# YonghaoHe/LFD-A-Light-and-Fast-Detector

Measured on NVIDIA H100. Metric: images/sec WIDERFACE-S inference 1280x720 batch=8 per GPU bf16, higher is better.
Workload: dtype bf16

## Files before the change

### lfd-a-light-and-fast-detector_b200/csrc/conv_umma.cu

```cuda
#include <stdlib.h>

#include <type_traits>

#include "conv_common.cuh"
#include "ptx.cuh"

namespace lfd {

static constexpr int kProdThreads = 128;
static constexpr int kConsumerThreads = 256;
static constexpr int kConvThreads = kConsumerThreads + kProdThreads;

#define LFD_LAMBDA_INLINE __attribute__((always_inline))

#ifdef LFD_B200_TRACE
#define LFD_TRACE(role, idx, slot) \
    do { if (p.trace && blockIdx.x == 0 && (idx) < 32) p.trace[((role) * 32 + (idx)) * 4 + (slot)] = clock64(); } while (0)
#define LFD_TRACE_EPI(tr, idx, slot) \
    do { if ((tr) && blockIdx.x == 0 && (idx) < 16) (tr)[(idx) * 8 + (slot)] = clock64(); } while (0)
#else
#define LFD_TRACE(role, idx, slot) ((void)0)
#define LFD_TRACE_EPI(tr, idx, slot) ((void)0)
#endif

// ... 541 lines not shown
                        const uint2 pe = *reinterpret_cast<const uint2*>(tp);
                        cp_async16_full(dst_cc + pe.y, src + pe.x);
                    }
                } else {
#pragma unroll 2
                    for (int pxi = px0; pxi < p.n_px; pxi += pstep) {
                        const PxDelta pd = delta[pxi];
                        const int y = iy0 + pd.dy, x = ix0 + pd.dx;
                        const bool ok = ((unsigned)y < (unsigned)lg.H) && ((unsigned)x < (unsigned)lg.W);
                        cp_async16(dst_cc + table[pxi].dst_off, src_cc + (ok ? (y * p.W + x) : 0) * p.Cin, ok);
                    }
                }
                cp_async_mbar_arrive(&full[s]);
                if (ptid == 0) LFD_TRACE(0, it, 2);
            }
        }
        cp_async_wait_all();
        }
    }
    LFD_TL_END(p.tl);
}

static constexpr int kS4Rows = 67, kS4Cols = 36, kS4Pix = kS4Rows * kS4Cols;
static constexpr int kS4RowBytes = kS4Cols * 8;
static constexpr int kS4PatchBytes = kS4Pix * 8;
static constexpr int kS4PerThread = (kS4Pix + kProdThreads - 1) / kProdThreads;
static constexpr int kS4Batch = 5;
static constexpr int kS4Groups = kS4Rows * 10;
static constexpr int kS4GroupsPerThread = (kS4Groups + kProdThreads - 1) / kProdThreads;
static constexpr int kS4GroupBatch = 3;
static constexpr int kS4PatchOverrun = 768;
LFD_DEVINL constexpr int s4_slot(int a, int b) {
    return ((a & 1) ? ((b & 1) ? 0 : 147) : ((b & 1) ? 291 : 446)) + (a >> 1) * 9 + (b >> 1);
}
static constexpr int kS4Lbo = 599 * 16;
static constexpr int kS4Bar = 0;
static constexpr int kS4Shift = 256;
static constexpr int kS4Staging = 2048;
static constexpr int kS4W0 = kS4Staging + 2 * 8192;
static constexpr int kS4W1 = kS4W0 + 6144;
static constexpr int kS4W2 = kS4W1 + 8192;
static constexpr int kS4W3 = kS4W2 + 73728;
static constexpr int kS4Planes = kS4W3 + 8192;
static constexpr int kS4Ring = kS4Planes + 8 * kS4Lbo;
static constexpr int kS4Smem = kS4Ring + 2 * kS4PatchBytes + kS4PatchOverrun;
static constexpr int kS4WBytes = kS4Planes - kS4W0;
static_assert(kS4Smem <= 227 * 1024, "stem4 shared memory");

LFD_DEVINL void s4_block(int i, int& a0, int& b0, bool& packed) {
    packed = i == 8 || i == 13;
    a0 = packed ? 32 : 8 * (i < 8 ? i >> 1 : i - 9);
    b0 = i < 8 ? 1 + 8 * (i & 1) : (i == 8 ? 1 : 0);
}
LFD_DEVINL void s4_run(int num_tiles, int& t0, int& t1) {
    t0 = (int)((uint64_t)blockIdx.x * (uint32_t)num_tiles / gridDim.x);
    t1 = (int)((uint64_t)(blockIdx.x + 1) * (uint32_t)num_tiles / gridDim.x);
}

LFD_DEVINL void consumers_bar_sync() { asm volatile("bar.sync 3, 256;" ::: "memory"); }

template <bool F16, bool EXT>
__global__ void __launch_bounds__(kConvThreads, 1) stem4_kernel(const __grid_constant__ UmmaConvParams p) {
    extern __shared__ __align__(1024) uint8_t smem[];
    uint64_t* full = reinterpret_cast<uint64_t*>(smem + kS4Bar);
    uint64_t* empty = full + 2;
    uint64_t* wbar = empty + 2;
    uint64_t* res_bar = wbar + 1;
    float* shifts = reinterpret_cast<float*>(smem + kS4Shift);
    pdl_launch_dependents();
    LFD_TL_BEGIN(p.tl);
    const int tid = threadIdx.x;
    const int warp = tid >> 5;
    const int lane = tid & 31;
    if (tid == 0) {
        for (int i = 0; i < 2; ++i) {
            mbar_init(&full[i], kProdThreads);
            mbar_init(&empty[i], kConsumerThreads / 32);
        }
        mbar_init(wbar, 1);
        mbar_init(&res_bar[0], 1);
        mbar_init(&res_bar[1], 1);
        fence_mbar_init();
    }
    if (tid < 256) {
        const int k = tid >> 6;
        const float* s = k == 0 ? p.shift : (k == 1 ? p.shift2 : (k == 2 ? p.shift_s2 : p.shift_s3));
        shifts[tid] = s ? round16<F16>(s[tid & 63]) : 0.f;
    }
    __syncthreads();
    const LaunchGrid lg = launch_grid<MODE_STEM4, EXT>(p);

    if (warp < kConsumerThreads / 32) {
        asm volatile("setmaxnreg.inc.sync.aligned.u32 224;");
        const int wg = warp >> 2;
        if (tid == 0) {
            mbar_arrive_expect_tx(wbar, kS4WBytes);
            auto load_w = [&](uint32_t dst, const __nv_bfloat16* src, uint32_t bytes) LFD_LAMBDA_INLINE {
                for (uint32_t off = 0; off < bytes; off += 32768)
                    bulk_g2s(smem_u32(smem) + dst + off, reinterpret_cast<const uint8_t*>(src) + off, bytes - off < 32768 ? bytes - off : 32768, wbar);
            };
            load_w(kS4W0, p.w, kS4W1 - kS4W0);
            load_w(kS4W1, p.w2, kS4W2 - kS4W1);
            load_w(kS4W2, p.w_s2, kS4W3 - kS4W2);
            load_w(kS4W3, p.w_s3, kS4Planes - kS4W3);
        }
        pdl_wait();
        mbar_wait(wbar, 0);

        EpiCtx e;
        e.stg_bytes = 8192u;
        e.nbuf = 1;
        e.stg = smem_u32(smem + kS4Staging) + (uint32_t)wg * 8192u;
        e.r0 = (warp & 3) * 16 + (lane >> 2);
        e.tq = lane & 3;
        e.wtid = tid & 127;
        e.wg = wg;
        e.lane = lane;
#ifdef LFD_B200_TRACE
        e.tr = p.trace && e.wtid == 0 ? p.trace + (3 * 32 + wg) * 4 : nullptr;
#endif
        const float* sh0 = shifts;
        const float* sh1 = shifts + 64;
        const float* sh2 = shifts + 128;
        const float* sh3 = shifts + 192;
        const uint32_t planes = smem_u32(smem + kS4Planes);
        const uint64_t adesc_stem = wgmma_desc(0, 16, 2 * kS4RowBytes);
        const uint64_t adesc_row = wgmma_desc(0, 16, 8 * 16);
        const uint64_t b0desc = wgmma_desc(smem_u32(smem + kS4W0), 64 * 16, 128);
        const uint64_t b1desc = wgmma_desc(smem_u32(smem + kS4W1), 64 * 16, 128);
        const uint64_t b2desc = wgmma_desc(smem_u32(smem + kS4W2), 64 * 16, 128);
        const uint64_t b3desc = wgmma_desc(smem_u32(smem + kS4W3), 64 * 16, 128);
        const uint64_t adesc_pl = wgmma_desc(planes + (uint32_t)wg * 8u * 144u, kS4Lbo, 144);
        const int brow = 2 * (warp & 3), bcol = lane >> 2;
        const int sh = (lane >> 3) & 1, sc = lane & 7;

        const int H1 = EXT ? (lg.H - 1) / 2 + 1 : p.H1, W1 = EXT ? (lg.W - 1) / 2 + 1 : p.W1;
        int tile0, tile1;
        s4_run(lg.num_tiles, tile0, tile1);
        uint32_t store_count = 0, res_count = 0;
        for (int tile = tile0, lt = 0; tile < tile1; ++tile, ++lt) {
            const uint32_t s = lt & 1, ph = (lt >> 1) & 1;
            const int n = fast_div(tile, lg.magic_tpi);
            const int t = tile - n * lg.tiles_per_img;
            const int ty = fast_div(t, lg.magic_tx);
            const int tx = t - ty * lg.tiles_x;
            const int oy0 = ty * 16, ox0 = tx * 8;
            const bool inherit = tile > tile0 && tx > 0, pass_on = tile + 1 < tile1 && tx + 1 < lg.tiles_x;
            if (e.wtid == 0) LFD_TRACE(1 + wg, lt, 0);
            mbar_wait(&full[s], ph);
            if (e.wtid == 0) LFD_TRACE(1 + wg, lt, 1);
            fence_proxy_async_smem();
            const uint32_t patch = smem_u32(smem + kS4Ring) + s * kS4PatchBytes;

            const int nblk = inherit ? 9 : 14, half = (nblk + 1) >> 1;
            const int first = wg ? half : 0, cnt = wg ? nblk - half : half;
#pragma unroll 1
            for (int kp = 0; kp < (cnt + 1) >> 1; ++kp) {
                int blk[2] = {first + 2 * kp, first + min(2 * kp + 1, cnt - 1)};
                float c0[2][32];
                wgmma_fence_regs<32>(c0[0]);
                wgmma_fence_regs<32>(c0[1]);
                wgmma_fence();
#pragma unroll
                for (int q = 0; q < 2; ++q) {
                    int a0, b0;
                    bool packed;
                    s4_block(blk[q], a0, b0, packed);
                    const uint32_t boff = (uint32_t)(a0 * 2 * kS4RowBytes + b0 * 16);
                    const uint64_t ad = (packed ? adesc_row : adesc_stem) + ((patch + boff) >> 4);
#pragma unroll
                    for (int kh = 0; kh < 3; ++kh)
                        wgmma_ss<64, F16>(c0[q], ad + (uint32_t)(kh * kS4RowBytes / 16), b0desc + (uint32_t)(kh * 2 * 64 * 16 / 16), kh != 0);
                }
                wgmma_commit();
                wgmma_wait<0>();
                wgmma_fence_regs<32>(c0[0]);
                wgmma_fence_regs<32>(c0[1]);
                uint32_t a1[2][16];
#pragma unroll
                for (int q = 0; q < 2; ++q)
#pragma unroll
                    for (int kk = 0; kk < 4; ++kk) {
                        const int c = 16 * kk + 2 * e.tq;
#pragma unroll
                        for (int r = 0; r < 4; ++r) {
                            const float x0 = c0[q][8 * kk + 2 * r] + sh0[c + 8 * (r >> 1)], x1 = c0[q][8 * kk + 2 * r + 1] + sh0[c + 8 * (r >> 1) + 1];
                            a1[q][4 * kk + r] = p.relu ? pack2_relu<F16>(x0, x1) : pack2<F16>(x0, x1);
                        }
                    }
                float c1[2][32];
                wgmma_fence_regs<32>(c1[0]);
                wgmma_fence_regs<32>(c1[1]);
                wgmma_fence();
                tail_mma<64, 64, F16>(c1[0], a1[0], b1desc);
                tail_mma<64, 64, F16>(c1[1], a1[1], b1desc);
                wgmma_commit();
                wgmma_wait<0>();
                wgmma_fence_regs<32>(c1[0]);
                wgmma_fence_regs<32>(c1[1]);
                float2 bv[8];
#pragma unroll
                for (int j = 0; j < 8; ++j) bv[j] = *reinterpret_cast<const float2*>(sh1 + 8 * j + 2 * e.tq);
#pragma unroll
                for (int q = 0; q < 2; ++q) {
                    int a0, b0;
                    bool packed;
                    s4_block(blk[q], a0, b0, packed);
                    if (packed && (warp & 3)) continue;
                    uint32_t v[8][2];
#pragma unroll
                    for (int h = 0; h < 2; ++h) {
                        const int a = packed ? a0 : a0 + brow + h, b = b0 + bcol + (packed ? 8 * h : 0);
                        const int y1 = 2 * oy0 - 1 + a, x1 = 2 * ox0 - 1 + b;
                        const bool in = (unsigned)y1 < (unsigned)H1 && (unsigned)x1 < (unsigned)W1;
#pragma unroll
                        for (int j = 0; j < 8; ++j) {
                            const float x0 = c1[q][4 * j + 2 * h] + bv[j].x, x1v = c1[q][4 * j + 2 * h + 1] + bv[j].y;
                            const uint32_t w = p.relu2 ? pack2_relu<F16>(x0, x1v) : pack2<F16>(x0, x1v);
                            v[j][h] = in ? w : 0u;
                        }
                    }
                    const int a = packed ? a0 : a0 + brow + sh, b = b0 + sc + (packed ? 8 * sh : 0);
                    const uint32_t addr = planes + (uint32_t)s4_slot(a, b) * 16u + (uint32_t)(lane >> 4) * kS4Lbo;
#pragma unroll
                    for (int k = 0; k < 4; ++k)
                        stmatrix_x4(addr + (uint32_t)(2 * k * kS4Lbo), v[2 * k][0], v[2 * k][1], v[2 * k + 1][0], v[2 * k + 1][1]);
                }
            }
            __syncwarp();
            if (lane == 0) mbar_arrive(&empty[s]);
            if (e.wtid == 0) LFD_TRACE(1 + wg, lt, 2);
            fence_proxy_async_smem();
            consumers_bar_sync();
            if (e.wtid == 0) LFD_TRACE(1 + wg, lt, 3);

            float acc[32];
            wgmma_fence_regs<32>(acc);
            wgmma_fence();
#pragma unroll
            for (int k16 = 0; k16 < 4; ++k16)
#pragma unroll
                for (int tap = 0; tap < 9; ++tap)
                    wgmma_ss<64, F16>(acc, adesc_pl + (uint32_t)(k16 * 2 * kS4Lbo / 16 + s4_slot(tap / 3, tap % 3)),
                                      b2desc + (uint32_t)((tap * 8 + 2 * k16) * 64 * 16 / 16), (k16 | tap) != 0);
            wgmma_commit();
            wgmma_wait<0>();
            wgmma_fence_regs<32>(acc);
            consumers_bar_sync();
            if (pass_on) {
                const int rs = lane >> 3, a = 16 * wg + brow + (rs & 1) + 8 * (rs >> 1);
                const uint32_t src = planes + (uint32_t)(lane & 7) * kS4Lbo + (uint32_t)s4_slot(a, 16) * 16u;
                sts128(src - 8u * 16u, lds128(src));
                if (wg == 1 && brow == 0 && lane < 8) {
                    const uint32_t src32 = planes + (uint32_t)lane * kS4Lbo + (uint32_t)s4_slot(32, 16) * 16u;
                    sts128(src32 - 8u * 16u, lds128(src32));
                }
                __syncwarp();
            }
#ifdef LFD_B200_TRACE
            if (e.wtid == 0 && p.trace && blockIdx.x == 0 && lt < 16) p.trace[(3 * 32 + wg + 2 * lt) * 4 + 3] = clock64();
#endif

            uint32_t a2[16];
#pragma unroll
            for (int kk = 0; kk < 4; ++kk) {
                const int c = 16 * kk + 2 * e.tq;
#pragma unroll
                for (int r = 0; r < 4; ++r) {
                    const float x0 = acc[8 * kk + 2 * r] + sh2[c + 8 * (r >> 1)], x1 = acc[8 * kk + 2 * r + 1] + sh2[c + 8 * (r >> 1) + 1];
                    a2[4 * kk + r] = p.relu_s2 ? pack2_relu<F16>(x0, x1) : pack2<F16>(x0, x1);
                }
            }
            float acc2[32];
            wgmma_fence_regs<32>(acc2);
            wgmma_fence();
            tail_mma<64, 64, F16>(acc2, a2, b3desc);
            wgmma_commit();
            wgmma_wait<0>();
            wgmma_fence_regs<32>(acc2);
            store_tile<MODE_3X3S2, 64, F16>(e, acc2, 64, sh3, (bool)p.relu_s3, false, nullptr, &p.tm_out, &p.tm_res, ox0, oy0 + wg * 8, n,
                                            true, true, &res_bar[wg], store_count, res_count);
        }
        if (e.wtid == 0) bulk_wait_all();
    } else {
        asm volatile("setmaxnreg.dec.sync.aligned.u32 56;");
        const int ptid = tid - kConsumerThreads;
        const bool u8 = p.input_format == 1;
        const int plane = p.H * p.W;
        pdl_wait();
        int tile0, tile1;
        s4_run(lg.num_tiles, tile0, tile1);
        for (int tile = tile0, lt = 0; tile < tile1; ++tile, ++lt) {
            const uint32_t s = lt & 1, ph = (lt >> 1) & 1;
            const int n = fast_div(tile, lg.magic_tpi), t = tile - n * lg.tiles_per_img;
            const int ty = fast_div(t, lg.magic_tx);
            const int iy0 = 4 * 16 * ty - 3, ix0 = 4 * 8 * (t - ty * lg.tiles_x) - 3;
            const bool interior = iy0 >= 0 && ix0 >= 0 && iy0 + kS4Rows <= lg.H && ix0 + kS4Cols <= lg.W;
            if (ptid == 0) LFD_TRACE(0, lt, 0);
            mbar_wait(&empty[s], ph ^ 1);
            if (ptid == 0) LFD_TRACE(0, lt, 1);
            const uint32_t dst0 = smem_u32(smem + kS4Ring) + s * kS4PatchBytes;
            if (p.in_words) {
#pragma unroll 1
                for (int j0 = 0; j0 < kS4GroupsPerThread; j0 += kS4GroupBatch) {
                    uint32_t wd[kS4GroupBatch][3];
                    bool ok[kS4GroupBatch];
#pragma unroll
                    for (int j = 0; j < kS4GroupBatch; ++j) {
                        const int q = ptid + (j0 + j) * kProdThreads;
                        const int r = q / 10, g = q - r * 10;
                        const int y = iy0 + r, x = ix0 - 1 + 4 * g;
                        ok[j] = q < kS4Groups && (unsigned)y < (unsigned)lg.H && (unsigned)x < (unsigned)lg.W;
                        const uint32_t* src = reinterpret_cast<const uint32_t*>(reinterpret_cast<const uint8_t*>(p.in_raw) +
                                                                                ((ptrdiff_t)n * plane + (ptrdiff_t)y * p.W + x) * 3);
#pragma unroll
                        for (int k = 0; k < 3; ++k) wd[j][k] = ok[j] ? __ldg(src + k) : 0u;
                    }
#pragma unroll
                    for (int j = 0; j < kS4GroupBatch; ++j) {
                        const int q = ptid + (j0 + j) * kProdThreads;
                        if (q >= kS4Groups) break;
                        const int r = q / 10, g = q - r * 10;
                        const int in_cols = lg.W - (ix0 - 1 + 4 * g);
                        uint32_t px[4][2];
#pragma unroll
                        for (int k = 0; k < 4; ++k) {
                            float f[3];
                            const bool okk = ok[j] && (!EXT || k < in_cols);
#pragma unroll
                            for (int c = 0; c < 3; ++c) {
                                const uint32_t byte = (wd[j][(3 * k + c) >> 2] >> (8 * ((3 * k + c) & 3))) & 0xffu;
                                f[c] = okk ? ((float)byte - 127.5f) * (1.0f / 127.5f) : 0.f;
                            }
                            px[k][0] = pack2<F16>(f[0], f[1]);
                            px[k][1] = pack2<F16>(f[2], 0.f);
                        }
                        const uint32_t d = dst0 + (uint32_t)(r * kS4RowBytes + 32 * g);
                        if (g > 0) asm volatile("st.shared.v2.b32 [%0], {%1, %2};" ::"r"(d - 8u), "r"(px[0][0]), "r"(px[0][1]) : "memory");
                        if (g < 9) {
                            asm volatile("st.shared.v4.b32 [%0], {%1, %2, %3, %4};" ::"r"(d), "r"(px[1][0]), "r"(px[1][1]), "r"(px[2][0]),
                                         "r"(px[2][1]) : "memory");
                            asm volatile("st.shared.v2.b32 [%0], {%1, %2};" ::"r"(d + 16u), "r"(px[3][0]), "r"(px[3][1]) : "memory");
                        }
                    }
                }
            } else {
#pragma unroll 1
                for (int j0 = 0; j0 < kS4PerThread; j0 += kS4Batch) {
                    uint32_t raw[kS4Batch][3];
                    bool ok[kS4Batch];
#pragma unroll
                    for (int j = 0; j < kS4Batch; ++j) {
                        const int q = ptid + (j0 + j) * kProdThreads;
                        const int r = q / kS4Cols, c = q - r * kS4Cols;
                        const int y = iy0 + r, x = ix0 + c;
                        ok[j] = q < kS4Pix && (interior || ((unsigned)y < (unsigned)lg.H && (unsigned)x < (unsigned)lg.W));
                        const ptrdiff_t pix = ok[j] ? (ptrdiff_t)n * plane + (ptrdiff_t)y * p.W + x : 0;
                        if (u8) {
                            const uint8_t* src = reinterpret_cast<const uint8_t*>(p.in_raw) + pix * 3;
                            raw[j][0] = __ldg(src); raw[j][1] = __ldg(src + 1); raw[j][2] = __ldg(src + 2);
                        } else {
                            const float* src = reinterpret_cast<const float*>(p.in_raw) + (ok[j] ? (ptrdiff_t)n * 2 * plane + pix : 0);
                            raw[j][0] = __float_as_uint(__ldg(src)); raw[j][1] = __float_as_uint(__ldg(src + plane));
                            raw[j][2] = __float_as_uint(__ldg(src + 2 * plane));
                        }
                    }
#pragma unroll
                    for (int j = 0; j < kS4Batch; ++j) {
                        const int q = ptid + (j0 + j) * kProdThreads;
                        if (q >= kS4Pix) break;
                        float f[3];
#pragma unroll
                        for (int k = 0; k < 3; ++k) {
                            f[k] = u8 ? ((float)raw[j][k] - 127.5f) * (1.0f / 127.5f) : __uint_as_float(raw[j][k]);
                            if (!ok[j]) f[k] = 0.f;
                        }
                        const uint32_t lo = pack2<F16>(f[0], f[1]), hi = pack2<F16>(f[2], 0.f);
                        asm volatile("st.shared.v2.b32 [%0], {%1, %2};" ::"r"(dst0 + q * 8), "r"(lo), "r"(hi) : "memory");
                    }
                }
            }
// ... 283 lines not shown
```

### lfd-a-light-and-fast-detector_b200/csrc/ptx.cuh

```cuda
#pragma once
#include <cuda_runtime.h>
#include <cuda_bf16.h>
#include <cuda_fp16.h>
#include <stdint.h>

namespace lfd {

#define LFD_DEVINL __device__ __forceinline__

#ifndef LFD_SPIN_LIMIT
#define LFD_SPIN_LIMIT (1u << 27)
#endif

LFD_DEVINL uint32_t smem_u32(const void* p) { return (uint32_t)__cvta_generic_to_shared(p); }

LFD_DEVINL void mbar_init(uint64_t* bar, uint32_t count) {
    asm volatile("mbarrier.init.shared::cta.b64 [%0], %1;" ::"r"(smem_u32(bar)), "r"(count));
}
LFD_DEVINL void fence_mbar_init() { asm volatile("fence.mbarrier_init.release.cluster;" ::: "memory"); }
LFD_DEVINL void mbar_arrive(uint64_t* bar) {
    asm volatile("mbarrier.arrive.shared::cta.b64 _, [%0];" ::"r"(smem_u32(bar)) : "memory");
}
LFD_DEVINL void mbar_arrive_expect_tx(uint64_t* bar, uint32_t bytes) {
    asm volatile("mbarrier.arrive.expect_tx.shared::cta.b64 _, [%0], %1;" ::"r"(smem_u32(bar)), "r"(bytes) : "memory");
// ... 81 lines not shown
LFD_DEVINL void bulk_wait_all() { asm volatile("cp.async.bulk.wait_group 0;" ::: "memory"); }
template <int N>
LFD_DEVINL void bulk_wait_read() { asm volatile("cp.async.bulk.wait_group.read %0;" ::"n"(N) : "memory"); }

LFD_DEVINL uint64_t wgmma_desc(uint32_t smem_addr, uint32_t lbo_bytes, uint32_t sbo_bytes) {
    uint64_t d = 0;
    d |= (uint64_t)((smem_addr >> 4) & 0x3FFF);
    d |= (uint64_t)((lbo_bytes >> 4) & 0x3FFF) << 16;
    d |= (uint64_t)((sbo_bytes >> 4) & 0x3FFF) << 32;
    return d;
}
LFD_DEVINL void wgmma_fence() { asm volatile("wgmma.fence.sync.aligned;" ::: "memory"); }
LFD_DEVINL void wgmma_commit() { asm volatile("wgmma.commit_group.sync.aligned;" ::: "memory"); }
template <int N>
LFD_DEVINL void wgmma_wait() { asm volatile("wgmma.wait_group.sync.aligned %0;" ::"n"(N) : "memory"); }
template <int N>
LFD_DEVINL void wgmma_fence_regs(float* d) {
#pragma unroll
    for (int i = 0; i < N; ++i) asm volatile("" : "+f"(d[i])::"memory");
}

template <int N> struct Wgmma;
template <> struct Wgmma<16> {
    template <int TA, int TB>
    static LFD_DEVINL void ss_bf16(float* d, uint64_t a, uint64_t b, uint32_t acc) {
        asm volatile("{\n\t.reg .pred p;\n\tsetp.ne.b32 p, %10, 0;\n\t"
                     "wgmma.mma_async.sync.aligned.m64n16k16.f32.bf16.bf16 {%0, %1, %2, %3, %4, %5, %6, %7}, %8, %9, p, 1, 1, %11, %12;\n\t}"
                     : "+f"(d[0]), "+f"(d[1]), "+f"(d[2]), "+f"(d[3]), "+f"(d[4]), "+f"(d[5]), "+f"(d[6]), "+f"(d[7])
                     : "l"(a), "l"(b), "r"(acc), "n"(TA), "n"(TB));
    }
    template <int TA, int TB>
    static LFD_DEVINL void ss_f16(float* d, uint64_t a, uint64_t b, uint32_t acc) {
        asm volatile("{\n\t.reg .pred p;\n\tsetp.ne.b32 p, %10, 0;\n\t"
                     "wgmma.mma_async.sync.aligned.m64n16k16.f32.f16.f16 {%0, %1, %2, %3, %4, %5, %6, %7}, %8, %9, p, 1, 1, %11, %12;\n\t}"
                     : "+f"(d[0]), "+f"(d[1]), "+f"(d[2]), "+f"(d[3]), "+f"(d[4]), "+f"(d[5]), "+f"(d[6]), "+f"(d[7])
                     : "l"(a), "l"(b), "r"(acc), "n"(TA), "n"(TB));
    }
};
template <> struct Wgmma<32> {
    template <int TA, int TB>
    static LFD_DEVINL void ss_bf16(float* d, uint64_t a, uint64_t b, uint32_t acc) {
        asm volatile("{\n\t.reg .pred p;\n\tsetp.ne.b32 p, %18, 0;\n\t"
                     "wgmma.mma_async.sync.aligned.m64n32k16.f32.bf16.bf16 {%0, %1, %2, %3, %4, %5, %6, %7, %8, %9, %10, %11, %12, %13, %14, %15}, %16, %17, p, 1, 1, %19, %20;\n\t}"
                     : "+f"(d[0]), "+f"(d[1]), "+f"(d[2]), "+f"(d[3]), "+f"(d[4]), "+f"(d[5]), "+f"(d[6]), "+f"(d[7]), "+f"(d[8]), "+f"(d[9]), "+f"(d[10]), "+f"(d[11]), "+f"(d[12]), "+f"(d[13]), "+f"(d[14]), "+f"(d[15])
                     : "l"(a), "l"(b), "r"(acc), "n"(TA), "n"(TB));
    }
    template <int TA, int TB>
    static LFD_DEVINL void ss_f16(float* d, uint64_t a, uint64_t b, uint32_t acc) {
        asm volatile("{\n\t.reg .pred p;\n\tsetp.ne.b32 p, %18, 0;\n\t"
                     "wgmma.mma_async.sync.aligned.m64n32k16.f32.f16.f16 {%0, %1, %2, %3, %4, %5, %6, %7, %8, %9, %10, %11, %12, %13, %14, %15}, %16, %17, p, 1, 1, %19, %20;\n\t}"
                     : "+f"(d[0]), "+f"(d[1]), "+f"(d[2]), "+f"(d[3]), "+f"(d[4]), "+f"(d[5]), "+f"(d[6]), "+f"(d[7]), "+f"(d[8]), "+f"(d[9]), "+f"(d[10]), "+f"(d[11]), "+f"(d[12]), "+f"(d[13]), "+f"(d[14]), "+f"(d[15])
                     : "l"(a), "l"(b), "r"(acc), "n"(TA), "n"(TB));
    }
};
template <> struct Wgmma<64> {
    template <int TA, int TB>
    static LFD_DEVINL void ss_bf16(float* d, uint64_t a, uint64_t b, uint32_t acc) {
        asm volatile("{\n\t.reg .pred p;\n\tsetp.ne.b32 p, %34, 0;\n\t"
                     "wgmma.mma_async.sync.aligned.m64n64k16.f32.bf16.bf16 {%0, %1, %2, %3, %4, %5, %6, %7, %8, %9, %10, %11, %12, %13, %14, %15, %16, %17, %18, %19, %20, %21, %22, %23, %24, %25, %26, %27, %28, %29, %30, %31}, %32, %33, p, 1, 1, %35, %36;\n\t}"
                     : "+f"(d[0]), "+f"(d[1]), "+f"(d[2]), "+f"(d[3]), "+f"(d[4]), "+f"(d[5]), "+f"(d[6]), "+f"(d[7]), "+f"(d[8]), "+f"(d[9]), "+f"(d[10]), "+f"(d[11]), "+f"(d[12]), "+f"(d[13]), "+f"(d[14]), "+f"(d[15]), "+f"(d[16]), "+f"(d[17]), "+f"(d[18]), "+f"(d[19]), "+f"(d[20]), "+f"(d[21]), "+f"(d[22]), "+f"(d[23]), "+f"(d[24]), "+f"(d[25]), "+f"(d[26]), "+f"(d[27]), "+f"(d[28]), "+f"(d[29]), "+f"(d[30]), "+f"(d[31])
                     : "l"(a), "l"(b), "r"(acc), "n"(TA), "n"(TB));
    }
    template <int TA, int TB>
    static LFD_DEVINL void ss_f16(float* d, uint64_t a, uint64_t b, uint32_t acc) {
        asm volatile("{\n\t.reg .pred p;\n\tsetp.ne.b32 p, %34, 0;\n\t"
                     "wgmma.mma_async.sync.aligned.m64n64k16.f32.f16.f16 {%0, %1, %2, %3, %4, %5, %6, %7, %8, %9, %10, %11, %12, %13, %14, %15, %16, %17, %18, %19, %20, %21, %22, %23, %24, %25, %26, %27, %28, %29, %30, %31}, %32, %33, p, 1, 1, %35, %36;\n\t}"
                     : "+f"(d[0]), "+f"(d[1]), "+f"(d[2]), "+f"(d[3]), "+f"(d[4]), "+f"(d[5]), "+f"(d[6]), "+f"(d[7]), "+f"(d[8]), "+f"(d[9]), "+f"(d[10]), "+f"(d[11]), "+f"(d[12]), "+f"(d[13]), "+f"(d[14]), "+f"(d[15]), "+f"(d[16]), "+f"(d[17]), "+f"(d[18]), "+f"(d[19]), "+f"(d[20]), "+f"(d[21]), "+f"(d[22]), "+f"(d[23]), "+f"(d[24]), "+f"(d[25]), "+f"(d[26]), "+f"(d[27]), "+f"(d[28]), "+f"(d[29]), "+f"(d[30]), "+f"(d[31])
                     : "l"(a), "l"(b), "r"(acc), "n"(TA), "n"(TB));
    }
};
template <> struct Wgmma<128> {
    template <int TA, int TB>
    static LFD_DEVINL void ss_bf16(float* d, uint64_t a, uint64_t b, uint32_t acc) {
        asm volatile("{\n\t.reg .pred p;\n\tsetp.ne.b32 p, %66, 0;\n\t"
                     "wgmma.mma_async.sync.aligned.m64n128k16.f32.bf16.bf16 {%0, %1, %2, %3, %4, %5, %6, %7, %8, %9, %10, %11, %12, %13, %14, %15, %16, %17, %18, %19, %20, %21, %22, %23, %24, %25, %26, %27, %28, %29, %30, %31, %32, %33, %34, %35, %36, %37, %38, %39, %40, %41, %42, %43, %44, %45, %46, %47, %48, %49, %50, %51, %52, %53, %54, %55, %56, %57, %58, %59, %60, %61, %62, %63}, %64, %65, p, 1, 1, %67, %68;\n\t}"
                     : "+f"(d[0]), "+f"(d[1]), "+f"(d[2]), "+f"(d[3]), "+f"(d[4]), "+f"(d[5]), "+f"(d[6]), "+f"(d[7]), "+f"(d[8]), "+f"(d[9]), "+f"(d[10]), "+f"(d[11]), "+f"(d[12]), "+f"(d[13]), "+f"(d[14]), "+f"(d[15]), "+f"(d[16]), "+f"(d[17]), "+f"(d[18]), "+f"(d[19]), "+f"(d[20]), "+f"(d[21]), "+f"(d[22]), "+f"(d[23]), "+f"(d[24]), "+f"(d[25]), "+f"(d[26]), "+f"(d[27]), "+f"(d[28]), "+f"(d[29]), "+f"(d[30]), "+f"(d[31]), "+f"(d[32]), "+f"(d[33]), "+f"(d[34]), "+f"(d[35]), "+f"(d[36]), "+f"(d[37]), "+f"(d[38]), "+f"(d[39]), "+f"(d[40]), "+f"(d[41]), "+f"(d[42]), "+f"(d[43]), "+f"(d[44]), "+f"(d[45]), "+f"(d[46]), "+f"(d[47]), "+f"(d[48]), "+f"(d[49]), "+f"(d[50]), "+f"(d[51]), "+f"(d[52]), "+f"(d[53]), "+f"(d[54]), "+f"(d[55]), "+f"(d[56]), "+f"(d[57]), "+f"(d[58]), "+f"(d[59]), "+f"(d[60]), "+f"(d[61]), "+f"(d[62]), "+f"(d[63])
                     : "l"(a), "l"(b), "r"(acc), "n"(TA), "n"(TB));
    }
    template <int TA, int TB>
    static LFD_DEVINL void ss_f16(float* d, uint64_t a, uint64_t b, uint32_t acc) {
        asm volatile("{\n\t.reg .pred p;\n\tsetp.ne.b32 p, %66, 0;\n\t"
                     "wgmma.mma_async.sync.aligned.m64n128k16.f32.f16.f16 {%0, %1, %2, %3, %4, %5, %6, %7, %8, %9, %10, %11, %12, %13, %14, %15, %16, %17, %18, %19, %20, %21, %22, %23, %24, %25, %26, %27, %28, %29, %30, %31, %32, %33, %34, %35, %36, %37, %38, %39, %40, %41, %42, %43, %44, %45, %46, %47, %48, %49, %50, %51, %52, %53, %54, %55, %56, %57, %58, %59, %60, %61, %62, %63}, %64, %65, p, 1, 1, %67, %68;\n\t}"
                     : "+f"(d[0]), "+f"(d[1]), "+f"(d[2]), "+f"(d[3]), "+f"(d[4]), "+f"(d[5]), "+f"(d[6]), "+f"(d[7]), "+f"(d[8]), "+f"(d[9]), "+f"(d[10]), "+f"(d[11]), "+f"(d[12]), "+f"(d[13]), "+f"(d[14]), "+f"(d[15]), "+f"(d[16]), "+f"(d[17]), "+f"(d[18]), "+f"(d[19]), "+f"(d[20]), "+f"(d[21]), "+f"(d[22]), "+f"(d[23]), "+f"(d[24]), "+f"(d[25]), "+f"(d[26]), "+f"(d[27]), "+f"(d[28]), "+f"(d[29]), "+f"(d[30]), "+f"(d[31]), "+f"(d[32]), "+f"(d[33]), "+f"(d[34]), "+f"(d[35]), "+f"(d[36]), "+f"(d[37]), "+f"(d[38]), "+f"(d[39]), "+f"(d[40]), "+f"(d[41]), "+f"(d[42]), "+f"(d[43]), "+f"(d[44]), "+f"(d[45]), "+f"(d[46]), "+f"(d[47]), "+f"(d[48]), "+f"(d[49]), "+f"(d[50]), "+f"(d[51]), "+f"(d[52]), "+f"(d[53]), "+f"(d[54]), "+f"(d[55]), "+f"(d[56]), "+f"(d[57]), "+f"(d[58]), "+f"(d[59]), "+f"(d[60]), "+f"(d[61]), "+f"(d[62]), "+f"(d[63])
                     : "l"(a), "l"(b), "r"(acc), "n"(TA), "n"(TB));
    }
};
template <int N> struct WgmmaRs;
template <> struct WgmmaRs<16> {
    static LFD_DEVINL void rs_bf16(float* d, const uint32_t* a, uint64_t b, uint32_t acc) {
        asm volatile("{\n\t.reg .pred p;\n\tsetp.ne.b32 p, %13, 0;\n\t"
                     "wgmma.mma_async.sync.aligned.m64n16k16.f32.bf16.bf16 {%0, %1, %2, %3, %4, %5, %6, %7}, {%8, %9, %10, %11}, %12, p, 1, 1, 0;\n\t}"
                     : "+f"(d[0]), "+f"(d[1]), "+f"(d[2]), "+f"(d[3]), "+f"(d[4]), "+f"(d[5]), "+f"(d[6]), "+f"(d[7])
                     : "r"(a[0]), "r"(a[1]), "r"(a[2]), "r"(a[3]), "l"(b), "r"(acc));
    }
    static LFD_DEVINL void rs_f16(float* d, const uint32_t* a, uint64_t b, uint32_t acc) {
        asm volatile("{\n\t.reg .pred p;\n\tsetp.ne.b32 p, %13, 0;\n\t"
                     "wgmma.mma_async.sync.aligned.m64n16k16.f32.f16.f16 {%0, %1, %2, %3, %4, %5, %6, %7}, {%8, %9, %10, %11}, %12, p, 1, 1, 0;\n\t}"
                     : "+f"(d[0]), "+f"(d[1]), "+f"(d[2]), "+f"(d[3]), "+f"(d[4]), "+f"(d[5]), "+f"(d[6]), "+f"(d[7])
                     : "r"(a[0]), "r"(a[1]), "r"(a[2]), "r"(a[3]), "l"(b), "r"(acc));
    }
};
template <> struct WgmmaRs<32> {
    static LFD_DEVINL void rs_bf16(float* d, const uint32_t* a, uint64_t b, uint32_t acc) {
        asm volatile("{\n\t.reg .pred p;\n\tsetp.ne.b32 p, %21, 0;\n\t"
                     "wgmma.mma_async.sync.aligned.m64n32k16.f32.bf16.bf16 {%0, %1, %2, %3, %4, %5, %6, %7, %8, %9, %10, %11, %12, %13, %14, %15}, {%16, %17, %18, %19}, %20, p, 1, 1, 0;\n\t}"
                     : "+f"(d[0]), "+f"(d[1]), "+f"(d[2]), "+f"(d[3]), "+f"(d[4]), "+f"(d[5]), "+f"(d[6]), "+f"(d[7]), "+f"(d[8]), "+f"(d[9]), "+f"(d[10]), "+f"(d[11]), "+f"(d[12]), "+f"(d[13]), "+f"(d[14]), "+f"(d[15])
                     : "r"(a[0]), "r"(a[1]), "r"(a[2]), "r"(a[3]), "l"(b), "r"(acc));
    }
    static LFD_DEVINL void rs_f16(float* d, const uint32_t* a, uint64_t b, uint32_t acc) {
        asm volatile("{\n\t.reg .pred p;\n\tsetp.ne.b32 p, %21, 0;\n\t"
                     "wgmma.mma_async.sync.aligned.m64n32k16.f32.f16.f16 {%0, %1, %2, %3, %4, %5, %6, %7, %8, %9, %10, %11, %12, %13, %14, %15}, {%16, %17, %18, %19}, %20, p, 1, 1, 0;\n\t}"
                     : "+f"(d[0]), "+f"(d[1]), "+f"(d[2]), "+f"(d[3]), "+f"(d[4]), "+f"(d[5]), "+f"(d[6]), "+f"(d[7]), "+f"(d[8]), "+f"(d[9]), "+f"(d[10]), "+f"(d[11]), "+f"(d[12]), "+f"(d[13]), "+f"(d[14]), "+f"(d[15])
                     : "r"(a[0]), "r"(a[1]), "r"(a[2]), "r"(a[3]), "l"(b), "r"(acc));
    }
};
template <> struct WgmmaRs<64> {
    static LFD_DEVINL void rs_bf16(float* d, const uint32_t* a, uint64_t b, uint32_t acc) {
        asm volatile("{\n\t.reg .pred p;\n\tsetp.ne.b32 p, %37, 0;\n\t"
                     "wgmma.mma_async.sync.aligned.m64n64k16.f32.bf16.bf16 {%0, %1, %2, %3, %4, %5, %6, %7, %8, %9, %10, %11, %12, %13, %14, %15, %16, %17, %18, %19, %20, %21, %22, %23, %24, %25, %26, %27, %28, %29, %30, %31}, {%32, %33, %34, %35}, %36, p, 1, 1, 0;\n\t}"
                     : "+f"(d[0]), "+f"(d[1]), "+f"(d[2]), "+f"(d[3]), "+f"(d[4]), "+f"(d[5]), "+f"(d[6]), "+f"(d[7]), "+f"(d[8]), "+f"(d[9]), "+f"(d[10]), "+f"(d[11]), "+f"(d[12]), "+f"(d[13]), "+f"(d[14]), "+f"(d[15]), "+f"(d[16]), "+f"(d[17]), "+f"(d[18]), "+f"(d[19]), "+f"(d[20]), "+f"(d[21]), "+f"(d[22]), "+f"(d[23]), "+f"(d[24]), "+f"(d[25]), "+f"(d[26]), "+f"(d[27]), "+f"(d[28]), "+f"(d[29]), "+f"(d[30]), "+f"(d[31])
                     : "r"(a[0]), "r"(a[1]), "r"(a[2]), "r"(a[3]), "l"(b), "r"(acc));
    }
    static LFD_DEVINL void rs_f16(float* d, const uint32_t* a, uint64_t b, uint32_t acc) {
        asm volatile("{\n\t.reg .pred p;\n\tsetp.ne.b32 p, %37, 0;\n\t"
                     "wgmma.mma_async.sync.aligned.m64n64k16.f32.f16.f16 {%0, %1, %2, %3, %4, %5, %6, %7, %8, %9, %10, %11, %12, %13, %14, %15, %16, %17, %18, %19, %20, %21, %22, %23, %24, %25, %26, %27, %28, %29, %30, %31}, {%32, %33, %34, %35}, %36, p, 1, 1, 0;\n\t}"
                     : "+f"(d[0]), "+f"(d[1]), "+f"(d[2]), "+f"(d[3]), "+f"(d[4]), "+f"(d[5]), "+f"(d[6]), "+f"(d[7]), "+f"(d[8]), "+f"(d[9]), "+f"(d[10]), "+f"(d[11]), "+f"(d[12]), "+f"(d[13]), "+f"(d[14]), "+f"(d[15]), "+f"(d[16]), "+f"(d[17]), "+f"(d[18]), "+f"(d[19]), "+f"(d[20]), "+f"(d[21]), "+f"(d[22]), "+f"(d[23]), "+f"(d[24]), "+f"(d[25]), "+f"(d[26]), "+f"(d[27]), "+f"(d[28]), "+f"(d[29]), "+f"(d[30]), "+f"(d[31])
                     : "r"(a[0]), "r"(a[1]), "r"(a[2]), "r"(a[3]), "l"(b), "r"(acc));
    }
};
template <> struct WgmmaRs<128> {
    static LFD_DEVINL void rs_bf16(float* d, const uint32_t* a, uint64_t b, uint32_t acc) {
        asm volatile("{\n\t.reg .pred p;\n\tsetp.ne.b32 p, %69, 0;\n\t"
                     "wgmma.mma_async.sync.aligned.m64n128k16.f32.bf16.bf16 {%0, %1, %2, %3, %4, %5, %6, %7, %8, %9, %10, %11, %12, %13, %14, %15, %16, %17, %18, %19, %20, %21, %22, %23, %24, %25, %26, %27, %28, %29, %30, %31, %32, %33, %34, %35, %36, %37, %38, %39, %40, %41, %42, %43, %44, %45, %46, %47, %48, %49, %50, %51, %52, %53, %54, %55, %56, %57, %58, %59, %60, %61, %62, %63}, {%64, %65, %66, %67}, %68, p, 1, 1, 0;\n\t}"
                     : "+f"(d[0]), "+f"(d[1]), "+f"(d[2]), "+f"(d[3]), "+f"(d[4]), "+f"(d[5]), "+f"(d[6]), "+f"(d[7]), "+f"(d[8]), "+f"(d[9]), "+f"(d[10]), "+f"(d[11]), "+f"(d[12]), "+f"(d[13]), "+f"(d[14]), "+f"(d[15]), "+f"(d[16]), "+f"(d[17]), "+f"(d[18]), "+f"(d[19]), "+f"(d[20]), "+f"(d[21]), "+f"(d[22]), "+f"(d[23]), "+f"(d[24]), "+f"(d[25]), "+f"(d[26]), "+f"(d[27]), "+f"(d[28]), "+f"(d[29]), "+f"(d[30]), "+f"(d[31]), "+f"(d[32]), "+f"(d[33]), "+f"(d[34]), "+f"(d[35]), "+f"(d[36]), "+f"(d[37]), "+f"(d[38]), "+f"(d[39]), "+f"(d[40]), "+f"(d[41]), "+f"(d[42]), "+f"(d[43]), "+f"(d[44]), "+f"(d[45]), "+f"(d[46]), "+f"(d[47]), "+f"(d[48]), "+f"(d[49]), "+f"(d[50]), "+f"(d[51]), "+f"(d[52]), "+f"(d[53]), "+f"(d[54]), "+f"(d[55]), "+f"(d[56]), "+f"(d[57]), "+f"(d[58]), "+f"(d[59]), "+f"(d[60]), "+f"(d[61]), "+f"(d[62]), "+f"(d[63])
                     : "r"(a[0]), "r"(a[1]), "r"(a[2]), "r"(a[3]), "l"(b), "r"(acc));
    }
    static LFD_DEVINL void rs_f16(float* d, const uint32_t* a, uint64_t b, uint32_t acc) {
        asm volatile("{\n\t.reg .pred p;\n\tsetp.ne.b32 p, %69, 0;\n\t"
                     "wgmma.mma_async.sync.aligned.m64n128k16.f32.f16.f16 {%0, %1, %2, %3, %4, %5, %6, %7, %8, %9, %10, %11, %12, %13, %14, %15, %16, %17, %18, %19, %20, %21, %22, %23, %24, %25, %26, %27, %28, %29, %30, %31, %32, %33, %34, %35, %36, %37, %38, %39, %40, %41, %42, %43, %44, %45, %46, %47, %48, %49, %50, %51, %52, %53, %54, %55, %56, %57, %58, %59, %60, %61, %62, %63}, {%64, %65, %66, %67}, %68, p, 1, 1, 0;\n\t}"
                     : "+f"(d[0]), "+f"(d[1]), "+f"(d[2]), "+f"(d[3]), "+f"(d[4]), "+f"(d[5]), "+f"(d[6]), "+f"(d[7]), "+f"(d[8]), "+f"(d[9]), "+f"(d[10]), "+f"(d[11]), "+f"(d[12]), "+f"(d[13]), "+f"(d[14]), "+f"(d[15]), "+f"(d[16]), "+f"(d[17]), "+f"(d[18]), "+f"(d[19]), "+f"(d[20]), "+f"(d[21]), "+f"(d[22]), "+f"(d[23]), "+f"(d[24]), "+f"(d[25]), "+f"(d[26]), "+f"(d[27]), "+f"(d[28]), "+f"(d[29]), "+f"(d[30]), "+f"(d[31]), "+f"(d[32]), "+f"(d[33]), "+f"(d[34]), "+f"(d[35]), "+f"(d[36]), "+f"(d[37]), "+f"(d[38]), "+f"(d[39]), "+f"(d[40]), "+f"(d[41]), "+f"(d[42]), "+f"(d[43]), "+f"(d[44]), "+f"(d[45]), "+f"(d[46]), "+f"(d[47]), "+f"(d[48]), "+f"(d[49]), "+f"(d[50]), "+f"(d[51]), "+f"(d[52]), "+f"(d[53]), "+f"(d[54]), "+f"(d[55]), "+f"(d[56]), "+f"(d[57]), "+f"(d[58]), "+f"(d[59]), "+f"(d[60]), "+f"(d[61]), "+f"(d[62]), "+f"(d[63])
                     : "r"(a[0]), "r"(a[1]), "r"(a[2]), "r"(a[3]), "l"(b), "r"(acc));
    }
};
template <int N, bool F16, int TA = 0, int TB = 0>
LFD_DEVINL void wgmma_ss(float* d, uint64_t a, uint64_t b, uint32_t acc) {
    if (F16) Wgmma<N>::template ss_f16<TA, TB>(d, a, b, acc);
    else Wgmma<N>::template ss_bf16<TA, TB>(d, a, b, acc);
}
template <int N, bool F16>
LFD_DEVINL void wgmma_rs(float* d, const uint32_t* a, uint64_t b, uint32_t acc) {
    if (F16) WgmmaRs<N>::rs_f16(d, a, b, acc);
    else WgmmaRs<N>::rs_bf16(d, a, b, acc);
}
LFD_DEVINL void stmatrix_x4(uint32_t addr, uint32_t r0, uint32_t r1, uint32_t r2, uint32_t r3) {
    asm volatile("stmatrix.sync.aligned.m8n8.x4.shared.b16 [%0], {%1, %2, %3, %4};" ::"r"(addr), "r"(r0), "r"(r1), "r"(r2), "r"(r3) : "memory");
}

#ifdef LFD_B200_TIMELINE
LFD_DEVINL unsigned long long globaltimer_ns() {
    unsigned long long t;
    asm volatile("mov.u64 %0, %%globaltimer;" : "=l"(t));
    return t;
}
#define LFD_TL_BEGIN(tl) do { if ((tl) && threadIdx.x == 0) atomicMin((tl), globaltimer_ns()); } while (0)
#define LFD_TL_END(tl) do { if ((tl) && threadIdx.x == 0) atomicMax((tl) + 1, globaltimer_ns()); } while (0)
#else
#define LFD_TL_BEGIN(tl) ((void)0)
#define LFD_TL_END(tl) ((void)0)
#endif
LFD_DEVINL uint32_t pack_bf16x2(float lo, float hi) {
    __nv_bfloat162 v = __floats2bfloat162_rn(lo, hi);
    return *reinterpret_cast<uint32_t*>(&v);
}
LFD_DEVINL uint32_t pack_bf16x2_relu(float lo, float hi) {
    uint32_t d;
    asm("cvt.rn.relu.bf16x2.f32 %0, %1, %2;" : "=r"(d) : "f"(hi), "f"(lo));
    return d;
}
LFD_DEVINL void sts128(uint32_t addr, uint4 v) {
    asm volatile("st.shared.v4.b32 [%0], {%1, %2, %3, %4};" ::"r"(addr), "r"(v.x), "r"(v.y), "r"(v.z), "r"(v.w) : "memory");
}
LFD_DEVINL float lds32f(uint32_t addr) {
    float v;
    asm volatile("ld.shared.f32 %0, [%1];" : "=f"(v) : "r"(addr) : "memory");
    return v;
}
LFD_DEVINL uint4 lds128(uint32_t addr) {
    uint4 v;
    asm volatile("ld.shared.v4.b32 {%0, %1, %2, %3}, [%4];" : "=r"(v.x), "=r"(v.y), "=r"(v.z), "=r"(v.w) : "r"(addr) : "memory");
    return v;
}
LFD_DEVINL float bf16_lo(uint32_t v) { return __uint_as_float(v << 16); }
LFD_DEVINL float bf16_hi(uint32_t v) { return __uint_as_float(v & 0xFFFF0000u); }
LFD_DEVINL float bf16_round(float x) { return __bfloat162float(__float2bfloat16_rn(x)); }

LFD_DEVINL uint32_t pack_f16x2(float lo, float hi) {
    uint32_t d;
    asm("cvt.rn.satfinite.f16x2.f32 %0, %1, %2;" : "=r"(d) : "f"(hi), "f"(lo));
    return d;
}
LFD_DEVINL uint32_t pack_f16x2_relu(float lo, float hi) {
    uint32_t d;
    asm("cvt.rn.relu.satfinite.f16x2.f32 %0, %1, %2;" : "=r"(d) : "f"(hi), "f"(lo));
    return d;
}
LFD_DEVINL float f16_lo(uint32_t v) { return __half2float(__ushort_as_half((unsigned short)(v & 0xFFFFu))); }
LFD_DEVINL float f16_hi(uint32_t v) { return __half2float(__ushort_as_half((unsigned short)(v >> 16))); }
template <bool F16> LFD_DEVINL uint32_t pack2(float lo, float hi) { return F16 ? pack_f16x2(lo, hi) : pack_bf16x2(lo, hi); }
template <bool F16> LFD_DEVINL uint32_t pack2_relu(float lo, float hi) { return F16 ? pack_f16x2_relu(lo, hi) : pack_bf16x2_relu(lo, hi); }
template <bool F16> LFD_DEVINL float up_lo(uint32_t v) { return F16 ? f16_lo(v) : bf16_lo(v); }
template <bool F16> LFD_DEVINL float up_hi(uint32_t v) { return F16 ? f16_hi(v) : bf16_hi(v); }
template <bool F16> LFD_DEVINL float round16(float x) { return F16 ? __half2float(__float2half_rn(x)) : bf16_round(x); }
template <bool F16> LFD_DEVINL uint32_t bits16(float x) {
    return F16 ? (uint32_t)__half_as_ushort(__float2half_rn(x)) : (uint32_t)__bfloat16_as_ushort(__float2bfloat16_rn(x));
}
LFD_DEVINL float up_lo_rt(uint32_t v, bool f16) { return f16 ? f16_lo(v) : bf16_lo(v); }
LFD_DEVINL float up_hi_rt(uint32_t v, bool f16) { return f16 ? f16_hi(v) : bf16_hi(v); }
LFD_DEVINL uint32_t pack2_rt(float lo, float hi, bool f16) { return f16 ? pack_f16x2(lo, hi) : pack_bf16x2(lo, hi); }
LFD_DEVINL float round16_rt(float x, bool f16) { return f16 ? __half2float(__float2half_rn(x)) : bf16_round(x); }

}
```

Measured before the change: 10450.

## Software-pipeline stem conv0/conv1 wgmma chain across blocks with async waits

After: 10720, median of 6. +2.6%, better.

```diff
diff --git a/lfd-a-light-and-fast-detector_b200/csrc/conv_umma.cu b/lfd-a-light-and-fast-detector_b200/csrc/conv_umma.cu
--- a/lfd-a-light-and-fast-detector_b200/csrc/conv_umma.cu
+++ b/lfd-a-light-and-fast-detector_b200/csrc/conv_umma.cu
@@ -717,61 +717,52 @@
             fence_proxy_async_smem();
             const uint32_t patch = smem_u32(smem + kS4Ring) + s * kS4PatchBytes;
 
-            const int nblk = inherit ? 9 : 14, half = (nblk + 1) >> 1;
-            const int first = wg ? half : 0, cnt = wg ? nblk - half : half;
-#pragma unroll 1
-            for (int kp = 0; kp < (cnt + 1) >> 1; ++kp) {
-                int blk[2] = {first + 2 * kp, first + min(2 * kp + 1, cnt - 1)};
-                float c0[2][32];
-                wgmma_fence_regs<32>(c0[0]);
-                wgmma_fence_regs<32>(c0[1]);
-                wgmma_fence();
-#pragma unroll
-                for (int q = 0; q < 2; ++q) {
+            const uint32_t blocks = inherit ? (wg ? 0x87654u : 0x3210u) : (wg ? 0xCB87654u : 0xDA93210u);
+            auto stem01 = [&](auto nb) LFD_LAMBDA_INLINE {
+                constexpr int NB = decltype(nb)::value;
+                static_assert(NB >= 2, "stem0/1 pipeline depth");
+                float c0[2][32], c1[2][32];
+                uint32_t a1[2][16];
+                auto issue_s0 = [&](int k) LFD_LAMBDA_INLINE {
                     int a0, b0;
                     bool packed;
-                    s4_block(blk[q], a0, b0, packed);
-                    const uint32_t boff = (uint32_t)(a0 * 2 * kS4RowBytes + b0 * 16);
-                    const uint64_t ad = (packed ? adesc_row : adesc_stem) + ((patch + boff) >> 4);
-#pragma unroll
-                    for (int kh = 0; kh < 3; ++kh)
-                        wgmma_ss<64, F16>(c0[q], ad + (uint32_t)(kh * kS4RowBytes / 16), b0desc + (uint32_t)(kh * 2 * 64 * 16 / 16), kh != 0);
-                }
-                wgmma_commit();
-                wgmma_wait<0>();
-                wgmma_fence_regs<32>(c0[0]);
-                wgmma_fence_regs<32>(c0[1]);
-                uint32_t a1[2][16];
-#pragma unroll
-                for (int q = 0; q < 2; ++q)
+                    s4_block((blocks >> 4 * k) & 15, a0, b0, packed);
+                    const uint64_t ad = (packed ? adesc_row : adesc_stem) + ((patch + (uint32_t)(a0 * 2 * kS4RowBytes + b0 * 16)) >> 4);
+                    wgmma_fence();
+                    wgmma_ss64_first<F16>(c0[k & 1], ad, b0desc);
+#pragma unroll
+                    for (int kh = 1; kh < 3; ++kh)
+                        wgmma_ss<64, F16>(c0[k & 1], ad + (uint32_t)(kh * kS4RowBytes / 16), b0desc + (uint32_t)(kh * 2 * 64 * 16 / 16), 1);
+                    wgmma_commit();
+                };
+                auto issue_s1 = [&](int k) LFD_LAMBDA_INLINE {
+                    float* c = c0[k & 1];
+                    uint32_t* a = a1[k & 1];
+                    wgmma_fence_regs<32>(c);
 #pragma unroll
                     for (int kk = 0; kk < 4; ++kk) {
-                        const int c = 16 * kk + 2 * e.tq;
+                        const int ch = 16 * kk + 2 * e.tq;
 #pragma unroll
                         for (int r = 0; r < 4; ++r) {
-                            const float x0 = c0[q][8 * kk + 2 * r] + sh0[c + 8 * (r >> 1)], x1 = c0[q][8 * kk + 2 * r + 1] + sh0[c + 8 * (r >> 1) + 1];
-                            a1[q][4 * kk + r] = p.relu ? pack2_relu<F16>(x0, x1) : pack2<F16>(x0, x1);
+                            const float x0 = c[8 * kk + 2 * r] + sh0[ch + 8 * (r >> 1)], x1 = c[8 * kk + 2 * r + 1] + sh0[ch + 8 * (r >> 1) + 1];
+                            a[4 * kk + r] = p.relu ? pack2_relu<F16>(x0, x1) : pack2<F16>(x0, x1);
                         }
                     }
-                float c1[2][32];
-                wgmma_fence_regs<32>(c1[0]);
-                wgmma_fence_regs<32>(c1[1]);
-                wgmma_fence();
-                tail_mma<64, 64, F16>(c1[0], a1[0], b1desc);
-                tail_mma<64, 64, F16>(c1[1], a1[1], b1desc);
-                wgmma_commit();
-                wgmma_wait<0>();
-                wgmma_fence_regs<32>(c1[0]);
-                wgmma_fence_regs<32>(c1[1]);
-                float2 bv[8];
-#pragma unroll
-                for (int j = 0; j < 8; ++j) bv[j] = *reinterpret_cast<const float2*>(sh1 + 8 * j + 2 * e.tq);
-#pragma unroll
-                for (int q = 0; q < 2; ++q) {
+                    wgmma_fence();
+                    wgmma_rs64_first<F16>(c1[k & 1], a, b1desc);
+#pragma unroll
+                    for (int kk = 1; kk < 4; ++kk) wgmma_rs<64, F16>(c1[k & 1], a + 4 * kk, b1desc + (uint32_t)(kk * 2 * 64 * 16 / 16), 1);
+                    wgmma_commit();
+                };
+                auto store = [&](int k) LFD_LAMBDA_INLINE {
+                    float* c = c1[k & 1];
+                    wgmma_fence_regs<32>(c);
                     int a0, b0;
                     bool packed;
-                    s4_block(blk[q], a0, b0, packed);
-                    if (packed && (warp & 3)) continue;
+                    s4_block((blocks >> 4 * k) & 15, a0, b0, packed);
+                    float2 bv[8];
+#pragma unroll
+                    for (int j = 0; j < 8; ++j) bv[j] = *reinterpret_cast<const float2*>(sh1 + 8 * j + 2 * e.tq);
                     uint32_t v[8][2];
 #pragma unroll
                     for (int h = 0; h < 2; ++h) {
@@ -780,18 +771,39 @@
                         const bool in = (unsigned)y1 < (unsigned)H1 && (unsigned)x1 < (unsigned)W1;
 #pragma unroll
                         for (int j = 0; j < 8; ++j) {
-                            const float x0 = c1[q][4 * j + 2 * h] + bv[j].x, x1v = c1[q][4 * j + 2 * h + 1] + bv[j].y;
+                            const float x0 = c[4 * j + 2 * h] + bv[j].x, x1v = c[4 * j + 2 * h + 1] + bv[j].y;
                             const uint32_t w = p.relu2 ? pack2_relu<F16>(x0, x1v) : pack2<F16>(x0, x1v);
                             v[j][h] = in ? w : 0u;
                         }
                     }
                     const int a = packed ? a0 : a0 + brow + sh, b = b0 + sc + (packed ? 8 * sh : 0);
                     const uint32_t addr = planes + (uint32_t)s4_slot(a, b) * 16u + (uint32_t)(lane >> 4) * kS4Lbo;
-#pragma unroll
-                    for (int k = 0; k < 4; ++k)
-                        stmatrix_x4(addr + (uint32_t)(2 * k * kS4Lbo), v[2 * k][0], v[2 * k][1], v[2 * k + 1][0], v[2 * k + 1][1]);
-                }
-            }
+                    const bool keep = !packed || (warp & 3) == 0;
+#pragma unroll
+                    for (int j = 0; j < 4; ++j)
+                        stmatrix_x4_if(keep, addr + (uint32_t)(2 * j * kS4Lbo), v[2 * j][0], v[2 * j][1], v[2 * j + 1][0], v[2 * j + 1][1]);
+                };
+                issue_s0(0);
+                issue_s0(1);
+                wgmma_wait<1>();
+                issue_s1(0);
+#pragma unroll
+                for (int i = 0; i < NB; ++i) {
+                    if (i + 1 < NB) {
+                        wgmma_wait<1>();
+                        if (i + 2 < NB) issue_s0(i + 2);
+                        issue_s1(i + 1);
+                        if (i + 2 < NB) wgmma_wait<2>();
+                        else wgmma_wait<1>();
+                    } else {
+                        wgmma_wait<0>();
+                    }
+                    store(i);
+                }
+            };
+            if (!inherit) stem01(std::integral_constant<int, 7>());
+            else if (wg) stem01(std::integral_constant<int, 5>());
+            else stem01(std::integral_constant<int, 4>());
             __syncwarp();
             if (lane == 0) mbar_arrive(&empty[s]);
             if (e.wtid == 0) LFD_TRACE(1 + wg, lt, 2);
diff --git a/lfd-a-light-and-fast-detector_b200/csrc/ptx.cuh b/lfd-a-light-and-fast-detector_b200/csrc/ptx.cuh
--- a/lfd-a-light-and-fast-detector_b200/csrc/ptx.cuh
+++ b/lfd-a-light-and-fast-detector_b200/csrc/ptx.cuh
@@ -257,8 +257,40 @@
     if (F16) WgmmaRs<N>::rs_f16(d, a, b, acc);
     else WgmmaRs<N>::rs_bf16(d, a, b, acc);
 }
+#define LFD_WGMMA_D64_OUT                                                                                                               \
+    "=f"(d[0]), "=f"(d[1]), "=f"(d[2]), "=f"(d[3]), "=f"(d[4]), "=f"(d[5]), "=f"(d[6]), "=f"(d[7]), "=f"(d[8]), "=f"(d[9]), "=f"(d[10]), \
+        "=f"(d[11]), "=f"(d[12]), "=f"(d[13]), "=f"(d[14]), "=f"(d[15]), "=f"(d[16]), "=f"(d[17]), "=f"(d[18]), "=f"(d[19]),            \
+        "=f"(d[20]), "=f"(d[21]), "=f"(d[22]), "=f"(d[23]), "=f"(d[24]), "=f"(d[25]), "=f"(d[26]), "=f"(d[27]), "=f"(d[28]),            \
+        "=f"(d[29]), "=f"(d[30]), "=f"(d[31])
+#define LFD_WGMMA_D64_REGS                                                                                                              \
+    "{%0, %1, %2, %3, %4, %5, %6, %7, %8, %9, %10, %11, %12, %13, %14, %15, %16, %17, %18, %19, %20, %21, %22, %23, %24, %25, %26, %27, " \
+    "%28, %29, %30, %31}"
+template <bool F16>
+LFD_DEVINL void wgmma_ss64_first(float* d, uint64_t a, uint64_t b) {
+    if (F16)
+        asm volatile("{\n\t.reg .pred p;\n\tsetp.ne.b32 p, 0, 0;\n\twgmma.mma_async.sync.aligned.m64n64k16.f32.f16.f16 " LFD_WGMMA_D64_REGS
+                     ", %32, %33, p, 1, 1, 0, 0;\n\t}" : LFD_WGMMA_D64_OUT : "l"(a), "l"(b));
+    else
+        asm volatile("{\n\t.reg .pred p;\n\tsetp.ne.b32 p, 0, 0;\n\twgmma.mma_async.sync.aligned.m64n64k16.f32.bf16.bf16 " LFD_WGMMA_D64_REGS
+                     ", %32, %33, p, 1, 1, 0, 0;\n\t}" : LFD_WGMMA_D64_OUT : "l"(a), "l"(b));
+}
+template <bool F16>
+LFD_DEVINL void wgmma_rs64_first(float* d, const uint32_t* a, uint64_t b) {
+    if (F16)
+        asm volatile("{\n\t.reg .pred p;\n\tsetp.ne.b32 p, 0, 0;\n\twgmma.mma_async.sync.aligned.m64n64k16.f32.f16.f16 " LFD_WGMMA_D64_REGS
+                     ", {%32, %33, %34, %35}, %36, p, 1, 1, 0;\n\t}" : LFD_WGMMA_D64_OUT : "r"(a[0]), "r"(a[1]), "r"(a[2]), "r"(a[3]), "l"(b));
+    else
+        asm volatile("{\n\t.reg .pred p;\n\tsetp.ne.b32 p, 0, 0;\n\twgmma.mma_async.sync.aligned.m64n64k16.f32.bf16.bf16 " LFD_WGMMA_D64_REGS
+                     ", {%32, %33, %34, %35}, %36, p, 1, 1, 0;\n\t}" : LFD_WGMMA_D64_OUT : "r"(a[0]), "r"(a[1]), "r"(a[2]), "r"(a[3]), "l"(b));
+}
+#undef LFD_WGMMA_D64_OUT
+#undef LFD_WGMMA_D64_REGS
 LFD_DEVINL void stmatrix_x4(uint32_t addr, uint32_t r0, uint32_t r1, uint32_t r2, uint32_t r3) {
     asm volatile("stmatrix.sync.aligned.m8n8.x4.shared.b16 [%0], {%1, %2, %3, %4};" ::"r"(addr), "r"(r0), "r"(r1), "r"(r2), "r"(r3) : "memory");
+}
+LFD_DEVINL void stmatrix_x4_if(bool on, uint32_t addr, uint32_t r0, uint32_t r1, uint32_t r2, uint32_t r3) {
+    asm volatile("{\n\t.reg .pred p;\n\tsetp.ne.b32 p, %5, 0;\n\t@p stmatrix.sync.aligned.m8n8.x4.shared.b16 [%0], {%1, %2, %3, %4};\n\t}"
+                 ::"r"(addr), "r"(r0), "r"(r1), "r"(r2), "r"(r3), "r"((uint32_t)on) : "memory");
 }
 
 #ifdef LFD_B200_TIMELINE
```
